# JulHoltzDevelopers/WavesAndEigenvalues.jl

Measured on AMD Instinct MI355X. Metric: eigenpairs/sec, higher is better.
Workload: dtype f64

## Files before the change

wavesandeigenvalues.jl_amd/csrc/debug.hip:

```cpp
#include <algorithm>

#include "family.h"

namespace {
struct StreamGuard {
    hipStream_t s = nullptr;
    ~StreamGuard() { if (s) (void)hipStreamDestroy(s); }
};
int64_t span(int64_t nv, int64_t stride, int64_t blk) { return nv > 0 ? (nv - 1) * stride + blk : 0; }
}

extern "C" int wae_debug_vec(int32_t device, int32_t op, const int64_t *sz, int32_t nsz, double *const *bufs, const int64_t *lens, int32_t nbuf,
                             const uint8_t *cmask, const int32_t *perm, int32_t *status_out) {
    return guarded([&]() {
        WAE_REQUIRE(sz && nsz >= 2 && nsz <= 16 && nbuf >= 0 && nbuf <= 16 && (nbuf == 0 || (bufs && lens)), "bad argument");
        int ndev = 0;
        HIP_CHECK(hipGetDeviceCount(&ndev));
        WAE_REQUIRE(device >= 0 && device < ndev, "no such device");
        for (int i = 0; i < nsz; ++i) WAE_REQUIRE(sz[i] >= 0 && sz[i] <= ((int64_t)1 << 31), "a size is negative or too large");
        for (int i = 0; i < nbuf; ++i) WAE_REQUIRE(lens[i] >= 0 && lens[i] <= ((int64_t)1 << 31), "a buffer length is negative or too large");
        auto S = [&](int i) -> int64_t { WAE_REQUIRE(i < nsz, "too few sizes for this operation"); return sz[i]; };
        WAE_REQUIRE(op != WAE_VEC_DENSE || sz[0] <= 2048, "dense coarse level too large (n > 2048)");
        HIP_CHECK(hipSetDevice(device));
        StreamGuard sg;
// ... 14 lines not shown
        const int64_t blk = n * nb;
        auto mask = [&]() -> const unsigned char * {
            if (!cmask) return nullptr;
            cm.upload(cmask, (size_t)(nb + 7) / 8, st);
            return cm.p;
        };
        auto count_of = [&](int i) -> int { const int64_t v = S(i); WAE_REQUIRE(v <= 4096, "a count is too large"); return (int)v; };
        auto want_partial = [&]() { partial.alloc((size_t)std::max(1024 * 32, 768 * 35) * (size_t)nb); return partial.p; };
        switch (op) {
        case WAE_VEC_DOTS: {
            const int nv = count_of(2);
            const int64_t stride = S(3);
            const cplx *V = need(0, span(nv, stride, blk)), *W = need(1, blk), *scale = opt(3, (int64_t)nv * nb);
            cplx *out = need(2, (int64_t)nv * nb);
            if (scale) launch_dots_scaled(V, (size_t)stride, nv, W, n, (int)nb, want_partial(), out, scale, st, mask());
            else launch_dots(V, (size_t)stride, nv, W, n, (int)nb, want_partial(), out, st, mask());
            break;
        }
        case WAE_VEC_NORMS:
            launch_norms(need(0, blk), n, (int)nb, want_partial(), need(1, nb), st, mask());
            break;
        case WAE_VEC_DOTS_MULTI: {
            const int nv = count_of(2), nw = count_of(3);
            WAE_REQUIRE(nw >= 1 && nw <= 4, "nw in 1..4");
            const cplx *V = need(0, span(nv, S(4), blk)), *W = need(1, span(nw, S(5), blk));
            launch_dots_multi(V, (size_t)S(4), nv, W, (size_t)S(5), nw, n, (int)nb, want_partial(), need(2, (int64_t)nv * nw * nb), st);
            break;
        }
        case WAE_VEC_AXPY_NEG: case WAE_VEC_LINCOMB: case WAE_VEC_LINCOMB_ADD: {
            const int nv = count_of(2);
            const cplx *V = need(0, span(nv, S(3), blk)), *c = need(1, (int64_t)nv * nb);
            cplx *W = need(2, blk);
            if (op == WAE_VEC_AXPY_NEG) launch_axpy_neg(V, (size_t)S(3), nv, c, W, n, (int)nb, st, mask());
            else if (op == WAE_VEC_LINCOMB) launch_lincomb(V, (size_t)S(3), nv, c, W, n, (int)nb, st);
            else launch_lincomb_add(V, (size_t)S(3), nv, c, W, n, (int)nb, st);
            break;
        }
        case WAE_VEC_AXPY_NEG_NORM: {
            const int nv = count_of(2);
            const cplx *V = need(0, span(nv, S(3), blk)), *h = need(1, (int64_t)nv * nb), *base = opt(4, blk);
            cplx *W = need(2, blk), *norms = need(3, nb), *inv = opt(5, nb);
            launch_axpy_neg_norm(V, (size_t)S(3), nv, h, W, n, (int)nb, want_partial(), norms, st, mask(), base, inv);
            break;
        }
        case WAE_VEC_AXPY_NEG_MULTI: {
            const int nv = count_of(2), cnt = count_of(4);
            WAE_REQUIRE(nv >= 1 && cnt >= 1 && cnt <= 4, "nv >= 1, cnt in 1..4");
            const cplx *V = need(0, span(nv, S(3), blk)), *h = need(1, (int64_t)nv * cnt * nb);
            launch_axpy_neg_multi(V, (size_t)S(3), nv, h, need(2, span(cnt, S(5), blk)), (size_t)S(5), cnt, n, (int)nb, st);
// ... 86 lines not shown
```

wavesandeigenvalues.jl_amd/csrc/family.h:

```cpp
#pragma once
#include <algorithm>
#include <chrono>
#include <future>

#include "amg.h"
#include "tiles.h"

struct RbState {
    cplx *Q = nullptr;
    int cap = 0, l = 0, S = 0;
    std::vector<int> kact;
    std::vector<zc> Hk;
    std::vector<zc> g;
    DevBuf<cplx> W, Vi, hb, alpha, alpha2, ycoef;
    std::future<void> w_job;
    void wait_w() { if (w_job.valid()) w_job.get(); }
    bool vi_valid = false;
    ~RbState() { if (w_job.valid()) w_job.wait(); }
};

struct wae_family {
    bool vc_light = false;
    int device = 0;
    hipStream_t stream = nullptr;
    int64_t d = 0;
    int T = 0;
    std::vector<int> term_plane;
    std::vector<zc> term_scale;
    std::vector<int64_t> term_nnz;
    int nplanes = 0;
    std::vector<CsrZ> planes0;
    std::vector<int> perm_h;
    DevBuf<int> perm_dev;
    std::vector<int> tile_row_ptr;
    const int *perm() const { return perm_dev.p; }
    std::vector<LevelOp> ops;
// ... 37 lines not shown
    size_t h_pin_pair_n = 0;
    size_t pc_stride_level = 0;
    ~wae_family() {
        if (stream) (void)hipStreamSynchronize(stream);
        if (h_pinned) (void)hipHostFree(h_pinned);
        if (h_pin_pair) (void)hipHostFree(h_pin_pair);
        if (stream) (void)hipStreamDestroy(stream);
    }
};

struct Batch {
    int nb;
    int cps;
    int nsys;
    int op;
};

static int env_int(const char *name, int dflt) { const char *v = getenv(name); return v ? atoi(v) : dflt; }
static bool xfer_tiles_on() { return env_int("WAE_XFER_TILES", 1) != 0; }
static double now_s() { return std::chrono::duration<double>(std::chrono::steady_clock::now().time_since_epoch()).count(); }
static void require_solver(const wae_family *h) {
    if (!h->solver_ready) throw WaeError(WAE_ERR_INVALID, "wae_solver_setup has not been called");
}
static void plane_coeffs(const wae_family *h, const double *coeffs, int op, std::vector<zc> &pc) {
    pc.assign(h->nplanes, zc(0));
    for (int k = 0; k < h->T; ++k) pc[h->term_plane[k]] += h->term_scale[k] * zc(coeffs[2 * k], coeffs[2 * k + 1]);
    if (op == WAE_OP_C)
        for (auto &c : pc) c = std::conj(c);
}

template <class F> static int guarded(F &&f) {
    try {
        return f();
    } catch (const WaeError &e) {
        wae_set_error(e.what());
        return e.code;
    } catch (const std::bad_alloc &) {
        wae_set_error("out of host memory");
        return WAE_ERR_INVALID;
    } catch (const std::exception &e) {
        wae_set_error(e.what());
        return WAE_ERR_INVALID;
    }
}
```

wavesandeigenvalues.jl_amd/csrc/lib.hip:

```cpp
#include <cmath>

#include "family.h"

static thread_local std::string g_last_error;
void wae_set_error(const std::string &m) { g_last_error = m; }

int wae_internal_device(const wae_family *h) { return h->device; }
hipStream_t wae_internal_stream(const wae_family *h) { return h->stream; }

static void upload_pc(wae_family *h, const std::vector<std::vector<zc>> &pcs) {
    const int nsys = (int)pcs.size();
    const int nl = (int)h->ops.size();
    const size_t per_level = (size_t)nsys * h->nplanes;
    std::vector<cplx> tab(per_level * (nl + 2));
    for (int l = 0; l <= nl + 1; ++l) {
        if (l >= nl && h->n_penalty == 0) break;
        const std::vector<int> &sp = l < nl ? h->slot_plane[l] : (l == nl ? h->pen_slot : h->pen_row_slot);
        for (int s = 0; s < nsys; ++s)
            for (int q = 0; q < h->nplanes; ++q) {
                const zc c = pcs[s][sp[q]];
                tab[l * per_level + (size_t)s * h->nplanes + q] = cplx{c.real(), c.imag()};
            }
    }
    h->pc_stride_level = per_level;
// ... 770 lines not shown
    for (int k = n - 1; k >= 0; --k) {
        if (dead[k]) { b[k] = 0; continue; }
        zc sres = b[k];
        for (int j = k + 1; j < n; ++j) sres -= A[(size_t)j * n + k] * b[j];
        b[k] = sres / A[(size_t)k * n + k];
    }
}

static void rb_d2h(wae_family *h, const cplx *src, cplx *dst, size_t cnt) {
    HIP_CHECK(hipMemcpyAsync(dst, src, cnt * sizeof(cplx), hipMemcpyDeviceToHost, h->stream));
    HIP_CHECK(hipStreamSynchronize(h->stream));
}

static void rb_reset(wae_family *h, cplx *Q, int cap, int l, const double *table, int npts, const cplx *Vinter) {
    RbState &R = h->rb;
    const int T = h->T;
    R.Q = Q; R.cap = cap; R.l = l; R.S = 0;
    R.kact.clear();
    for (int k = 0; k < T; ++k) {
        bool used = false;
        for (int p = 0; p < npts && !used; ++p) used = table[((size_t)p * T + k) * 2] != 0.0 || table[((size_t)p * T + k) * 2 + 1] != 0.0;
        if (used) R.kact.push_back(k);
    }
    const size_t vecl = (size_t)h->d * l;
    R.wait_w();
    if (R.W.n < R.kact.size() * (size_t)cap * vecl) {
        const size_t need = R.kact.size() * (size_t)cap * vecl;
        const int dev = h->device;
        RbState *Rp = &R;
        R.w_job = std::async(std::launch::async, [Rp, need, dev]() {
            HIP_CHECK(hipSetDevice(dev));
            Rp->W.alloc(need);
        });
    }
    R.Hk.assign(R.kact.size() * (size_t)cap * cap * l, zc(0));
    R.g.assign((size_t)cap * l, zc(0));
    if (R.Vi.n < vecl) R.Vi.alloc(vecl);
    HIP_CHECK(hipMemcpyAsync(R.Vi.p, Vinter, vecl * sizeof(cplx), hipMemcpyDeviceToDevice, h->stream));
    R.vi_valid = true;
    if (R.hb.n < (size_t)4 * (cap + 4) * l) R.hb.alloc((size_t)4 * (cap + 4) * l);
    if (R.alpha.n < (size_t)l) R.alpha.alloc(l);
    if (R.alpha2.n < (size_t)cap * l) R.alpha2.alloc((size_t)cap * l);
}

static void rb_append_block(wae_family *h, int cnt, const std::vector<std::vector<std::vector<zc>>> &pck) {
    RbState &R = h->rb;
    hipStream_t st = h->stream;
    const int64_t d = h->d;
    const int l = R.l, cap = R.cap, S = R.S;
    const size_t vecl = (size_t)d * l;
    std::vector<cplx> hh((size_t)(S + cnt) * cnt * l), n0((size_t)cnt * l), n1(l);
    const OpDev A0 = h->ops[0].dev(WAE_OP_N);
    cplx *qn = R.Q + (size_t)S * vecl;
    for (int j = 0; j < cnt; ++j) launch_norms(qn + (size_t)j * vecl, d, l, h->partial.p, R.hb.p + (size_t)j * l, st);
    rb_d2h(h, R.hb.p, n0.data(), (size_t)cnt * l);
    static const bool multi_axpy = !(getenv("WAE_RB_MULTI_AXPY") && atoi(getenv("WAE_RB_MULTI_AXPY")) == 0);
    const bool fits = (size_t)S * cnt * l * sizeof(cplx) <= 60 * 1024;
    for (int pass = 0; pass < 2 && S > 0; ++pass) {
        launch_dots_multi(R.Q, vecl, S, qn, vecl, cnt, d, l, h->partial.p, R.hb.p, st);
        if (multi_axpy && fits) {
            launch_axpy_neg_multi(R.Q, vecl, S, R.hb.p, qn, vecl, cnt, d, l, st);
            continue;
        }
        rb_d2h(h, R.hb.p, hh.data(), (size_t)S * cnt * l);
        std::vector<cplx> cj((size_t)S * l);
        for (int j = 0; j < cnt; ++j) {
            for (int i = 0; i < S; ++i)
                for (int c = 0; c < l; ++c) cj[(size_t)i * l + c] = hh[((size_t)i * cnt + j) * l + c];
            R.alpha2.upload(cj.data(), cj.size(), st);
            launch_axpy_neg(R.Q, vecl, S, R.alpha2.p, qn + (size_t)j * vecl, d, l, st);
            HIP_CHECK(hipStreamSynchronize(st));
        }
    }
    for (int j = 0; j < cnt; ++j) {
        cplx *q = qn + (size_t)j * vecl;
        for (int pass = 0; pass < 2 && j > 0; ++pass) {
            launch_dots(qn, vecl, j, q, d, l, h->partial.p, R.hb.p, st);
            launch_axpy_neg(qn, vecl, j, R.hb.p, q, d, l, st);
        }
        launch_norms(q, d, l, h->partial.p, R.hb.p, st);
        rb_d2h(h, R.hb.p, n1.data(), l);
        for (int c = 0; c < l; ++c) {
            const double nrm0 = n0[(size_t)j * l + c].x;
            n1[c] = (n1[c].x > 1e-9 * nrm0 && nrm0 > 0.0) ? cplx{n1[c].x, 0.0} : cplx{0.0, 0.0};
        }
        R.alpha.upload(n1.data(), l, st);
        launch_scale_inv(q, R.alpha.p, q, d, l, st);
        HIP_CHECK(hipStreamSynchronize(st));
    }
    launch_dots_multi(qn, vecl, cnt, R.Vi.p, vecl, 1, d, l, h->partial.p, R.hb.p, st);
    rb_d2h(h, R.hb.p, hh.data(), (size_t)cnt * l);
    for (int j = 0; j < cnt; ++j)
        for (int c = 0; c < l; ++c) R.g[(size_t)(S + j) * l + c] = zc(hh[(size_t)j * l + c].x, hh[(size_t)j * l + c].y);
    for (size_t ki = 0; ki < R.kact.size(); ++ki) {
        R.wait_w();
        cplx *Wk = R.W.p + ki * (size_t)cap * vecl;
        cplx *wn = Wk + (size_t)S * vecl;
        upload_pc(h, pck[ki]);
        for (int j = 0; j < cnt; ++j)
            launch_spmv(A0, pc_level(h, 0), l, qn + (size_t)j * vecl, wn + (size_t)j * vecl, nullptr, 0.0, l, MODE_AX, st);
        zc *H = &R.Hk[ki * (size_t)cap * cap * l];
        launch_dots_multi(R.Q, vecl, S + cnt, wn, vecl, cnt, d, l, h->partial.p, R.hb.p, st);
        rb_d2h(h, R.hb.p, hh.data(), (size_t)(S + cnt) * cnt * l);
        for (int i = 0; i < S + cnt; ++i)
            for (int j = 0; j < cnt; ++j)
                for (int c = 0; c < l; ++c) {
                    const cplx v = hh[((size_t)i * cnt + j) * l + c];
                    H[((size_t)(S + j) * cap + i) * l + c] = zc(v.x, v.y);
                }
        zc herm_factor(0);
        bool herm = false;
        {
            static const bool herm_on = !(getenv("WAE_RB_HERMITIAN") && atoi(getenv("WAE_RB_HERMITIAN")) == 0);
            const int kterm = R.kact[ki], pl = h->term_plane[kterm];
            const LevelOp &L0 = h->ops[0];
            for (size_t g = 0; g < L0.groups.size() && herm_on && !herm; ++g)
                for (int q = 0; q < L0.groups[g].nplanes; ++q)
                    if (h->slot_plane[0][(size_t)L0.groups[g].plane0 + q] == pl && L0.groups[g].symmetric && L0.groups[g].is_real) {
                        const zc sc = h->term_scale[kterm];
                        if (sc != zc(0)) { herm = true; herm_factor = sc / std::conj(sc); }
                    }
        }
        if (S > 0 && herm) {
            for (int i = 0; i < S; ++i)
                for (int j = 0; j < cnt; ++j)
                    for (int c = 0; c < l; ++c)
                        H[((size_t)i * cap + S + j) * l + c] = herm_factor * std::conj(H[((size_t)(S + j) * cap + i) * l + c]);
        } else if (S > 0) {
            launch_dots_multi(Wk, vecl, S, qn, vecl, cnt, d, l, h->partial.p, R.hb.p, st);
            rb_d2h(h, R.hb.p, hh.data(), (size_t)S * cnt * l);
            for (int i = 0; i < S; ++i)
                for (int j = 0; j < cnt; ++j)
                    for (int c = 0; c < l; ++c) {
                        const cplx v = hh[((size_t)i * cnt + j) * l + c];
                        H[((size_t)i * cap + S + j) * l + c] = zc(v.x, -v.y);
                    }
        }
    }
    R.S += cnt;
}

static void rb_append(wae_family *h, int count) {
    RbState &R = h->rb;
    WAE_REQUIRE(R.S + count <= R.cap, "snapshot store is full");
    std::vector<std::vector<std::vector<zc>>> pck(R.kact.size());
    for (size_t ki = 0; ki < R.kact.size(); ++ki) {
        std::vector<double> ek((size_t)2 * h->T, 0.0);
        ek[(size_t)2 * R.kact[ki]] = 1.0;
        pck[ki].resize(1);
        plane_coeffs(h, ek.data(), WAE_OP_N, pck[ki][0]);
    }
    for (int done = 0; done < count; done += 4) rb_append_block(h, std::min(4, count - done), pck);
}

static std::vector<cplx> rb_guess_coeffs(const wae_family *h, const double *ct_chunk, int ns) {
    const RbState &R = h->rb;
    const int S = R.S, l = R.l, cap = R.cap, T = h->T, nb = ns * l;
    std::vector<cplx> Y((size_t)S * nb);
    std::vector<zc> Hs((size_t)S * S), rhs(S);
    for (int sy = 0; sy < ns; ++sy) {
        const double *ct = ct_chunk + (size_t)sy * 2 * T;
        for (int k = 0; k < T; ++k)
            if ((ct[2 * k] != 0.0 || ct[2 * k + 1] != 0.0) && std::find(R.kact.begin(), R.kact.end(), k) == R.kact.end())
                throw WaeError(WAE_ERR_INVALID, "a term outside the projected set has a non-zero coefficient: rebuild the basis (mode 1)");
        for (int c = 0; c < l; ++c) {
            std::fill(Hs.begin(), Hs.end(), zc(0));
            for (size_t ki = 0; ki < R.kact.size(); ++ki) {
                const zc ck(ct[2 * R.kact[ki]], ct[2 * R.kact[ki] + 1]);
                if (ck == zc(0)) continue;
                const zc *H = &R.Hk[ki * (size_t)cap * cap * l];
                for (int sc = 0; sc < S; ++sc)
                    for (int i = 0; i < S; ++i) Hs[(size_t)sc * S + i] += ck * H[((size_t)sc * cap + i) * l + c];
            }
            for (int i = 0; i < S; ++i) rhs[i] = R.g[(size_t)i * l + c];
            small_solve(Hs, rhs, S);
// ... 1392 lines not shown
```

wavesandeigenvalues.jl_amd/csrc/setup.hip:

```cpp
#include <atomic>
#include <cmath>
#include <exception>
#include <map>
#include <memory>
#include <tuple>

#include "family.h"

OpDev LevelOp::dev(int op) const {
    OpDev o;
    memset(&o, 0, sizeof(o));
    o.ngroups = (int)groups.size();
    o.nplanes_total = nplanes;
    o.n = n;
    o.diag = diag.p;
    o.conj_diag = (op == WAE_OP_C) ? 1 : 0;
    o.tiles = !tiles.ready ? nullptr : (op == WAE_OP_N || tiles.all_symmetric) ? &tiles.dev : (tiles.ready_t ? &tiles.dev_t : nullptr);
    {
        const LongRows &LR = (op == WAE_OP_N) ? long_n : long_t;
        o.nlong = LR.n;
        o.long_rows = LR.rows.p; o.long_ptr = LR.ptr.p; o.long_col = LR.col.p; o.long_slot = LR.slot.p;
        o.long_val = LR.val.p; o.long_acc = LR.acc.p; o.long_part = LR.part.p;
        o.long_conj = (op == WAE_OP_C) ? 1 : 0;
    }
// ... 793 lines not shown
        h->NB = (int)opt(6, 64);
        WAE_REQUIRE(h->NB >= 1 && h->NB <= 256, "batch width must be in 1..256");
        WAE_REQUIRE(h->restart >= 2 && h->restart <= 200, "restart must be in 2..200");
        excl = (uint64_t)opt(7, 0.0);
        plane_coeffs(h, coeffs_ref, WAE_OP_N, pc);
        if (excl) {
            std::vector<double> cs(coeffs_ref, coeffs_ref + (size_t)2 * h->T);
            for (int k = 0; k < h->T && k < 52; ++k)
                if (excl >> k & 1) cs[2 * k] = cs[2 * k + 1] = 0.0;
            plane_coeffs(h, cs.data(), WAE_OP_N, pc_shape);
        }
    }

    void drop_hierarchy() {
        h->ops.resize(1);
        h->slot_plane.resize(1);
        h->xfer.clear();
    }

    void reserve_device_memory() {
        const size_t vec = (size_t)h->d * h->NB, need = vec * (size_t)(h->restart + 1);
        const size_t hint_l = (size_t)opt(8, 0.0), hint_s = (size_t)opt(9, 0.0);
        const size_t need_q = hint_l > 0 && hint_s > 0 && hint_l <= (size_t)h->NB ? (size_t)h->d * hint_l * hint_s : 0;
        const size_t need_w = need_q * (size_t)h->nplanes;
        h->rb.wait_w();
        if (h->V.n == need && h->rbQ.n >= need_q && h->rb.W.n >= need_w) return;
        basis_job.f = std::async(std::launch::async, [this, need, need_q, need_w]() {
            HIP_CHECK(hipSetDevice(h->device));
            if (h->V.n != need) h->V.alloc(need);
            const bool new_q = h->rbQ.n < need_q, new_w = h->rb.W.n < need_w;
            if (new_q) h->rbQ.alloc(need_q);
            if (new_w) h->rb.W.alloc(need_w);
            if (new_q && need_q) HIP_CHECK(hipMemset(h->rbQ.p, 0, need_q * sizeof(cplx)));
            if (new_w && need_w) HIP_CHECK(hipMemset(h->rb.W.p, 0, need_w * sizeof(cplx)));
            HIP_CHECK(hipDeviceSynchronize());
        });
    }

    void coarsen() {
        std::vector<int> visit0;
        if (!h->perm_h.empty()) { visit0.resize(h->perm_h.size()); for (size_t i = 0; i < h->perm_h.size(); ++i) visit0[h->perm_h[i]] = (int)i; }
        const bool want_plan = env.tile_level1 && !h->tile_row_ptr.empty();
        amg_setup(h->planes0, pc, ao, lv, &pen, excl ? &pc_shape : nullptr, visit0.empty() ? nullptr : &visit0, [&](const AmgLevel &L) {
            if (!want_plan || l1_job.f.valid() || &L != &lv[0]) return;
            l1_job.f = std::async(std::launch::async, [this]() { l1.run(h, lv[0], env); });
        });
        t_amg1 = now_s();
// ... 147 lines not shown
```

wavesandeigenvalues.jl_amd/csrc/vec.hip:

```cpp
#include "kernel_helpers.h"

__global__ void fill_zero_kernel(cplx *X, size_t count) {
    for (size_t e = (size_t)blockIdx.x * 256 + threadIdx.x; e < count; e += (size_t)gridDim.x * 256) X[e] = cplx{0.0, 0.0};
}
void launch_fill_zero(cplx *X, size_t count, hipStream_t st) {
    if (!count) return;
    hipLaunchKernelGGL(fill_zero_kernel, dim3(grid_for(count)), dim3(256), 0, st, X, count);
    HIP_CHECK(hipGetLastError());
}
void launch_copy(const cplx *X, cplx *Y, size_t count, hipStream_t st) {
    if (!count) return;
    HIP_CHECK(hipMemcpyAsync(Y, X, count * sizeof(cplx), hipMemcpyDeviceToDevice, st));
}
__global__ void add_kernel(const cplx *__restrict__ X, cplx *__restrict__ Y, size_t count) {
    for (size_t e = (size_t)blockIdx.x * 256 + threadIdx.x; e < count; e += (size_t)gridDim.x * 256) {
        cplx a = X[e], b = Y[e];
        Y[e] = cplx{a.x + b.x, a.y + b.y};
    }
}
void launch_add(const cplx *X, cplx *Y, size_t count, hipStream_t st) {
    if (!count) return;
    hipLaunchKernelGGL(add_kernel, dim3(grid_for(count)), dim3(256), 0, st, X, Y, count);
    HIP_CHECK(hipGetLastError());
}

__device__ __forceinline__ cplx vadd(cplx a, cplx b) { return cplx{a.x + b.x, a.y + b.y}; }
__device__ __forceinline__ double vadd(double a, double b) { return a + b; }
__device__ __forceinline__ cplx vshfl_xor(cplx a, int m) { return cplx{__shfl_xor(a.x, m), __shfl_xor(a.y, m)}; }
__device__ __forceinline__ double vshfl_xor(double a, int m) { return __shfl_xor(a, m); }
template <bool POW2, int NT, class T>
__device__ __forceinline__ T block_colsum(T v, int nb, T *sm) {
    const int tid = threadIdx.x;
    if (POW2) {
        for (int m = 32; m >= nb; m >>= 1) v = vadd(v, vshfl_xor(v, m));
        if ((tid & 63) < nb) sm[(tid >> 6) * nb + (tid & 63)] = v;
    } else {
        sm[tid] = v;
    }
    __syncthreads();
    if (tid < nb) {
        const int terms = POW2 ? NT / 64 : NT / nb;
        v = sm[tid];
        for (int k = 1; k < terms; ++k) v = vadd(v, sm[k * nb + tid]);
    }
    __syncthreads();
    return v;
}
template <int EPB>
__device__ __forceinline__ cplx sum_partials(const cplx *__restrict__ partial, int nblk, int count) {
    __shared__ cplx sm[256];
    constexpr int NS = 256 / EPB;
    const int slice = threadIdx.x / EPB;
    const int e = blockIdx.x * EPB + threadIdx.x % EPB;
    cplx acc = {0.0, 0.0};
    if (e < count)
        for (int k = slice; k < nblk; k += NS) { const cplx p = partial[(size_t)k * count + e]; acc.x += p.x; acc.y += p.y; }
    sm[threadIdx.x] = acc;
    __syncthreads();
#pragma unroll
    for (int s = NS / 2; s >= 1; s >>= 1) {
        if (slice < s) { sm[threadIdx.x].x += sm[threadIdx.x + s * EPB].x; sm[threadIdx.x].y += sm[threadIdx.x + s * EPB].y; }
        __syncthreads();
    }
    return sm[threadIdx.x];
}

constexpr int DOT_BLOCKS = 1024;
template <int MAXV, bool POW2>
__global__ __launch_bounds__(256) void dots_kernel(const cplx *__restrict__ V, size_t stride, int nv, const cplx *__restrict__ W,
                                                   int64_t n, int nb, cplx *__restrict__ partial,
// ... 92 lines not shown
            for (int i = 0; i < MAXV; ++i) {
                if (i < nv) {
                    const cplx v = V[(size_t)i * sv + e];
#pragma unroll
                    for (int j = 0; j < NW; ++j) {
                        acc[i][j].x += v.x * w[j].x + v.y * w[j].y;
                        acc[i][j].y += v.x * w[j].y - v.y * w[j].x;
                    }
                }
            }
        }
    }
#pragma unroll
    for (int i = 0; i < MAXV; ++i) {
#pragma unroll
        for (int j = 0; j < NW; ++j) {
            if (i < nv && j < nw) {
                const cplx s = block_colsum<false, 256>(acc[i][j], nb, sm);
                if (tid < nb) partial[((size_t)blockIdx.x * nv * nw + (size_t)i * nw + j) * nb + tid] = s;
            }
        }
    }
}
void launch_dots_multi(const cplx *V, size_t sv, int nv, const cplx *W, size_t sw, int nw, int64_t n, int nb, cplx *partial, cplx *out,
                       hipStream_t st) {
    if (nb < 1 || nb > 256 || nw < 1 || nw > 4) throw WaeError(WAE_ERR_INVALID, "dots_multi: nb in 1..256, nw in 1..4");
    int done = 0;
    while (done < nv) {
        const int chunk = std::min(8, nv - done);
        const int nblk = 768;
        hipLaunchKernelGGL((dots_multi_kernel<8, 4>), dim3(nblk), dim3(256), 0, st, V + (size_t)done * sv, sv, chunk, W, sw, nw, n, nb, partial);
        HIP_CHECK(hipGetLastError());
        const int count = chunk * nw * nb;
        launch_reduce_partials(partial, nblk, count, out + (size_t)done * nw * nb, 0, st);
        done += chunk;
    }
}
void launch_dots(const cplx *V, size_t stride, int nv, const cplx *W, int64_t n, int nb, cplx *partial, cplx *out, hipStream_t st,
                 const unsigned char *cmask) {
    dots_impl(V, stride, nv, W, n, nb, partial, out, 0, st, cmask);
}
void launch_dots_scaled(const cplx *V, size_t stride, int nv, const cplx *W, int64_t n, int nb, cplx *partial, cplx *out, const cplx *scale,
                        hipStream_t st, const unsigned char *cmask) {
    dots_impl(V, stride, nv, W, n, nb, partial, out, 0, st, cmask, scale);
}
void launch_norms(const cplx *X, int64_t n, int nb, cplx *partial, cplx *out, hipStream_t st, const unsigned char *cmask) {
    dots_impl(X, 0, 1, X, n, nb, partial, out, 1, st, cmask);
}

// ... 405 lines not shown
                               n, nb, l, nsys, done ? 1 : 0);
        });
        return;
    }
    const unsigned grid = row_grid(n, nb, 256, 1, 2048).grid;
    for_coef_groups(nv, nb, [&](int done, int chunk, size_t shm) {
        hipLaunchKernelGGL(lincomb_rep_kernel, dim3(grid), dim3(256), shm, st, Q + (size_t)done * stride, stride, chunk, y + (size_t)done * nb, X, n,
                           nb, l, done ? 1 : 0);
    });
}
__global__ __launch_bounds__(256) void mask_cols_kernel(cplx *__restrict__ X, const cplx *__restrict__ keep, size_t total, int nb) {
    for (size_t e = (size_t)blockIdx.x * 256 + threadIdx.x; e < total; e += (size_t)gridDim.x * 256) {
        if (keep[e % nb].x == 0.0) X[e] = cplx{0.0, 0.0};
    }
}
void launch_mask_cols(cplx *X, const cplx *keep, int64_t n, int nb, hipStream_t st) {
    const size_t total = (size_t)n * nb;
    if (!total) return;
    hipLaunchKernelGGL(mask_cols_kernel, dim3(grid_for(total)), dim3(256), 0, st, X, keep, total, nb);
    HIP_CHECK(hipGetLastError());
}

__global__ __launch_bounds__(256) void scale_inv_kernel(const cplx *__restrict__ X, const cplx *__restrict__ alpha, cplx *__restrict__ Y, size_t total, int nb,
                                                        const unsigned char *__restrict__ cmask) {
    for (size_t e = (size_t)blockIdx.x * 256 + threadIdx.x; e < total; e += (size_t)gridDim.x * 256) {
        if (cmask && !cmask[(e % nb) >> 3]) continue;
        const double a = alpha[e % nb].x;
        const double s = (a > 1e-300) ? 1.0 / a : 0.0;
        const cplx x = X[e];
        Y[e] = cplx{x.x * s, x.y * s};
    }
}
void launch_scale_inv(const cplx *X, const cplx *alpha, cplx *Y, int64_t n, int nb, hipStream_t st, const unsigned char *cmask) {
    size_t total = (size_t)n * nb;
    if (!total) return;
    hipLaunchKernelGGL(scale_inv_kernel, dim3(grid_for(total)), dim3(256), 0, st, X, alpha, Y, total, nb, cmask);
    HIP_CHECK(hipGetLastError());
}

__global__ __launch_bounds__(256) void axpby1_kernel(cplx a, const cplx *x, cplx b, const cplx *y, cplx *out, size_t n, int conj_x) {
    for (size_t e = (size_t)blockIdx.x * 256 + threadIdx.x; e < n; e += (size_t)gridDim.x * 256) {
        cplx r = cmul(a, conj_x ? cconj(x[e]) : x[e]);
        cfma(r, b, y[e]);
        out[e] = r;
    }
}
void launch_axpby1(cplx a, const cplx *x, cplx b, const cplx *y, cplx *out, size_t n, hipStream_t st, int conj_x) {
    if (!n) return;
    hipLaunchKernelGGL(axpby1_kernel, dim3(grid_for(n)), dim3(256), 0, st, a, x, b, y, out, n, conj_x);
    HIP_CHECK(hipGetLastError());
}
__global__ __launch_bounds__(256) void colmajor_to_inter_kernel(const cplx *__restrict__ Xc, int64_t d, int r, cplx *__restrict__ Xi, int nb,
                                                                const int *__restrict__ perm) {
    const size_t total = (size_t)d * nb;
    for (size_t e = (size_t)blockIdx.x * 256 + threadIdx.x; e < total; e += (size_t)gridDim.x * 256) {
        const size_t row = e / nb;
        const int b = (int)(e - row * nb);
        const size_t src = perm ? (size_t)perm[row] : row;
        Xi[e] = (b < r) ? Xc[(size_t)b * d + src] : cplx{0.0, 0.0};
// ... 427 lines not shown
```

wavesandeigenvalues.jl_amd/csrc/wae_internal.h:

```cpp
#pragma once
#include <hip/hip_runtime.h>
#include <complex>
#include <cstdint>
#include <cstdio>
#include <cstring>
#include <stdexcept>
#include <string>
#include <vector>

#include "../../include/waehip.h"

typedef std::complex<double> zc;
typedef double2 cplx;

struct WaeError : std::runtime_error {
    int code;
    WaeError(int c, const std::string &m) : std::runtime_error(m), code(c) {}
};
void wae_set_error(const std::string &m);
int wae_internal_device(const wae_family *h);
hipStream_t wae_internal_stream(const wae_family *h);

#define HIP_CHECK(expr)                                                                                  \
    do {                                                                                                 \
// ... 192 lines not shown
void launch_jacobi0(const OpDev &op, const cplx *pc, int cps, const cplx *B, cplx *X, double jac_w, int nb, hipStream_t s,
                    const unsigned char *cmask = nullptr);
void launch_spmv_multi(const OpDev &op, const cplx *pc, const int *plane_col, const cplx *X, cplx *Y, int nb, hipStream_t s);

void launch_dense_assemble(const cplx *planes, int nplanes, int n, const cplx *pc, int nsys, int op,
                           cplx *Ainv, hipStream_t s);
void launch_dense_invert(cplx *Ainv, int n, int nsys, int *status, hipStream_t s);
void launch_dense_apply(const cplx *Ainv, int n, int cps, const cplx *X, cplx *Y, int nb, hipStream_t s, const unsigned char *cmask = nullptr);

void launch_fill_zero(cplx *X, size_t count, hipStream_t s);
void launch_copy(const cplx *X, cplx *Y, size_t count, hipStream_t s);
void launch_dots(const cplx *V, size_t stride, int nv, const cplx *W, int64_t n, int nb, cplx *partial, cplx *out, hipStream_t s,
                 const unsigned char *cmask = nullptr);
void launch_axpy_neg_multi(const cplx *V, size_t stride, int nv, const cplx *h, cplx *W, size_t wstride, int cnt, int64_t n, int nb, hipStream_t s);
void launch_axpy_neg(const cplx *V, size_t stride, int nv, const cplx *h, cplx *W, int64_t n, int nb, hipStream_t s,
                     const unsigned char *cmask = nullptr);
void launch_axpy_neg_norm(const cplx *V, size_t stride, int nv, const cplx *h, cplx *W, int64_t n, int nb, cplx *partial, cplx *norms,
                          hipStream_t s, const unsigned char *cmask = nullptr, const cplx *base = nullptr, cplx *inv_out = nullptr);
void launch_dots_scaled(const cplx *V, size_t stride, int nv, const cplx *W, int64_t n, int nb, cplx *partial, cplx *out, const cplx *scale,
                        hipStream_t s, const unsigned char *cmask = nullptr);
void launch_lincomb(const cplx *V, size_t stride, int nv, const cplx *y, cplx *Y, int64_t n, int nb, hipStream_t s);
void launch_lincomb_add(const cplx *V, size_t stride, int nv, const cplx *y, cplx *X, int64_t n, int nb, hipStream_t s);
void launch_norms(const cplx *X, int64_t n, int nb, cplx *partial, cplx *out, hipStream_t s, const unsigned char *cmask = nullptr);
void launch_scale_inv(const cplx *X, const cplx *alpha, cplx *Y, int64_t n, int nb, hipStream_t s, const unsigned char *cmask = nullptr);
void launch_axpby1(cplx a, const cplx *x, cplx b, const cplx *y, cplx *out, size_t n, hipStream_t s, int conj_x = 0);
void launch_add(const cplx *X, cplx *Y, size_t count, hipStream_t s);
void launch_colmajor_to_inter(const cplx *Xc, int64_t d, int r, cplx *Xi, int nb, hipStream_t s, const int *perm = nullptr);
void launch_inter_to_colmajor(const cplx *Xi, int nb, int64_t d, int r, cplx *Xc, hipStream_t s, const int *perm = nullptr);
void launch_replicate(const cplx *Vc, int64_t d, int l, cplx *Xi, int nb, hipStream_t s, const int *perm = nullptr);
void launch_prolong_add(const int *ptr, const int *col, const double *val, int64_t n, const cplx *Xc, cplx *X, int nb, hipStream_t s,
                        const unsigned char *cmask = nullptr);
void launch_dots_multi(const cplx *V, size_t sv, int nv, const cplx *W, size_t sw, int nw, int64_t n, int nb, cplx *partial, cplx *out,
                       hipStream_t s);
void launch_gather_rows(const cplx *X, const int *rows, int64_t nrows, int nb, cplx *out, hipStream_t s);
void launch_scatter_add_rows(const cplx *D, const int *rows, int64_t nrows, int nb, cplx *X, hipStream_t s);
void launch_extract_cols(const cplx *X, int nb, int off, int l, cplx *out, int64_t n, hipStream_t s);
void launch_lincomb_rep(const cplx *Q, size_t stride, int nv, const cplx *y, cplx *X, int64_t n, int nb, int l, hipStream_t s);
void launch_mask_cols(cplx *X, const cplx *keep, int64_t n, int nb, hipStream_t s);
void launch_beyn_accum(const cplx *Xi, int nb, int64_t d, int l, int nsys, const cplx *w, const cplx *z, int npow, cplx *A, hipStream_t s,
                       int lA = 0, int c0 = 0, const int *perm = nullptr);
void launch_pt_gemm_batch(const cplx *V, size_t stride, int k, const cplx *G, cplx *U, int64_t d, int T, int nb, hipStream_t s);
void launch_pt_spmv_batch(const OpDev &op, const cplx *pc, const int *plane_col, const cplx *U, int nin, cplx *Y, int nb, int accumulate,
                          hipStream_t s);
void launch_pt_axpby_cols(const cplx *coef, const cplx *x, const cplx *y, cplx *out, int64_t d, int nb, hipStream_t s);
void launch_pt_project(cplx *vk, const cplx *v0, const cplx *dots, int nd, int64_t d, int nb, hipStream_t s);
struct GmresDev {
    int nb, m, histcap;
    cplx *R;
    double *cs;
    cplx *sn;
    cplx *g;
    double *sv;
    cplx *vsq;
    int *conv, *steps, *iters, *histlen, *stalled;
    double *relres, *bnorm;
    double *hist;
// ... 17 lines not shown
```

Before: 4.364.

## Batch reduced-basis append projections and remove host round-trips

Restructures the reduced-basis snapshot append so the spmv results for up to four terms, together with the initial-vector projection, are projected against Q by a single new wide multi-RHS dots kernel. All results come back in one device-to-host copy instead of one per term. The norm thresholding moves into scale_inv on the device, which removes per-column syncs and uploads. For Hermitian terms, W storage keeps only the current block rather than the whole basis, which cuts memory. This adds a new kernel with larger partial buffers and more complex bookkeeping, and the non-fitting axpy path now allocates a temporary device buffer on every pass.

```diff
diff --git a/wavesandeigenvalues.jl_amd/csrc/debug.hip b/wavesandeigenvalues.jl_amd/csrc/debug.hip
--- a/wavesandeigenvalues.jl_amd/csrc/debug.hip
+++ b/wavesandeigenvalues.jl_amd/csrc/debug.hip
@@ -60,9 +60,10 @@
             break;
         case WAE_VEC_DOTS_MULTI: {
             const int nv = count_of(2), nw = count_of(3);
-            WAE_REQUIRE(nw >= 1 && nw <= 4, "nw in 1..4");
+            WAE_REQUIRE(nw >= 1 && nw <= DOTS_MAXW, "nw in 1..20");
             const cplx *V = need(0, span(nv, S(4), blk)), *W = need(1, span(nw, S(5), blk));
-            launch_dots_multi(V, (size_t)S(4), nv, W, (size_t)S(5), nw, n, (int)nb, want_partial(), need(2, (int64_t)nv * nw * nb), st);
+            partial.alloc(dots_multi_partial_count(nw, (int)nb));
+            launch_dots_multi(V, (size_t)S(4), nv, W, (size_t)S(5), nw, n, (int)nb, partial.p, need(2, (int64_t)nv * nw * nb), st);
             break;
         }
         case WAE_VEC_AXPY_NEG: case WAE_VEC_LINCOMB: case WAE_VEC_LINCOMB_ADD: {
diff --git a/wavesandeigenvalues.jl_amd/csrc/family.h b/wavesandeigenvalues.jl_amd/csrc/family.h
--- a/wavesandeigenvalues.jl_amd/csrc/family.h
+++ b/wavesandeigenvalues.jl_amd/csrc/family.h
@@ -12,6 +12,8 @@
     std::vector<int> kact;
     std::vector<zc> Hk;
     std::vector<zc> g;
+    std::vector<zc> herm;
+    std::vector<size_t> woff;
     DevBuf<cplx> W, Vi, hb, alpha, alpha2, ycoef;
     std::future<void> w_job;
     void wait_w() { if (w_job.valid()) w_job.get(); }
@@ -95,6 +97,22 @@
 static void require_solver(const wae_family *h) {
     if (!h->solver_ready) throw WaeError(WAE_ERR_INVALID, "wae_solver_setup has not been called");
 }
+constexpr int RB_BLOCK = 4;
+constexpr int RB_TERMS = 4;
+static bool plane_real_symmetric(const wae_family *h, int pl) {
+    const LevelOp &L0 = h->ops[0];
+    for (size_t g = 0; g < L0.groups.size(); ++g)
+        for (int q = 0; q < L0.groups[g].nplanes; ++q)
+            if (h->slot_plane[0][(size_t)L0.groups[g].plane0 + q] == pl && L0.groups[g].symmetric && L0.groups[g].is_real) return true;
+    return false;
+}
+static bool rb_term_hermitian(const wae_family *h, int kterm, zc *factor) {
+    static const bool herm_on = env_int("WAE_RB_HERMITIAN", 1) != 0;
+    const zc sc = h->term_scale[kterm];
+    if (!herm_on || sc == zc(0) || !plane_real_symmetric(h, h->term_plane[kterm])) return false;
+    *factor = sc / std::conj(sc);
+    return true;
+}
 static void plane_coeffs(const wae_family *h, const double *coeffs, int op, std::vector<zc> &pc) {
     pc.assign(h->nplanes, zc(0));
     for (int k = 0; k < h->T; ++k) pc[h->term_plane[k]] += h->term_scale[k] * zc(coeffs[2 * k], coeffs[2 * k + 1]);
diff --git a/wavesandeigenvalues.jl_amd/csrc/lib.hip b/wavesandeigenvalues.jl_amd/csrc/lib.hip
--- a/wavesandeigenvalues.jl_amd/csrc/lib.hip
+++ b/wavesandeigenvalues.jl_amd/csrc/lib.hip
@@ -816,10 +816,16 @@
         for (int p = 0; p < npts && !used; ++p) used = table[((size_t)p * T + k) * 2] != 0.0 || table[((size_t)p * T + k) * 2 + 1] != 0.0;
         if (used) R.kact.push_back(k);
     }
-    const size_t vecl = (size_t)h->d * l;
+    const size_t vecl = (size_t)h->d * l, nk = R.kact.size();
+    R.herm.assign(nk, zc(0));
+    R.woff.assign(nk, 0);
+    size_t need = 0;
+    for (size_t ki = 0; ki < nk; ++ki) {
+        R.woff[ki] = need;
+        need += (size_t)(rb_term_hermitian(h, R.kact[ki], &R.herm[ki]) ? RB_BLOCK : cap) * vecl;
+    }
     R.wait_w();
-    if (R.W.n < R.kact.size() * (size_t)cap * vecl) {
-        const size_t need = R.kact.size() * (size_t)cap * vecl;
+    if (R.W.n < need) {
         const int dev = h->device;
         RbState *Rp = &R;
         R.w_job = std::async(std::launch::async, [Rp, need, dev]() {
@@ -827,27 +833,29 @@
             Rp->W.alloc(need);
         });
     }
-    R.Hk.assign(R.kact.size() * (size_t)cap * cap * l, zc(0));
+    R.Hk.assign(nk * (size_t)cap * cap * l, zc(0));
     R.g.assign((size_t)cap * l, zc(0));
     if (R.Vi.n < vecl) R.Vi.alloc(vecl);
     HIP_CHECK(hipMemcpyAsync(R.Vi.p, Vinter, vecl * sizeof(cplx), hipMemcpyDeviceToDevice, h->stream));
     R.vi_valid = true;
-    if (R.hb.n < (size_t)4 * (cap + 4) * l) R.hb.alloc((size_t)4 * (cap + 4) * l);
+    const size_t hbn = (2 * nk * RB_BLOCK + 1) * (size_t)(cap + RB_BLOCK) * l;
+    if (R.hb.n < hbn) R.hb.alloc(hbn);
     if (R.alpha.n < (size_t)l) R.alpha.alloc(l);
     if (R.alpha2.n < (size_t)cap * l) R.alpha2.alloc((size_t)cap * l);
-}
-
-static void rb_append_block(wae_family *h, int cnt, const std::vector<std::vector<std::vector<zc>>> &pck) {
+    const size_t np = dots_multi_partial_count(RB_TERMS * RB_BLOCK + 1, l);
+    if (h->partial.n < np) h->partial.alloc(np);
+}
+
+static void rb_append_block(wae_family *h, int cnt) {
     RbState &R = h->rb;
     hipStream_t st = h->stream;
     const int64_t d = h->d;
     const int l = R.l, cap = R.cap, S = R.S;
-    const size_t vecl = (size_t)d * l;
-    std::vector<cplx> hh((size_t)(S + cnt) * cnt * l), n0((size_t)cnt * l), n1(l);
+    const size_t vecl = (size_t)d * l, nk = R.kact.size();
     const OpDev A0 = h->ops[0].dev(WAE_OP_N);
     cplx *qn = R.Q + (size_t)S * vecl;
-    for (int j = 0; j < cnt; ++j) launch_norms(qn + (size_t)j * vecl, d, l, h->partial.p, R.hb.p + (size_t)j * l, st);
-    rb_d2h(h, R.hb.p, n0.data(), (size_t)cnt * l);
+    cplx *n0 = R.alpha2.p;
+    for (int j = 0; j < cnt; ++j) launch_norms(qn + (size_t)j * vecl, d, l, h->partial.p, n0 + (size_t)j * l, st);
     static const bool multi_axpy = !(getenv("WAE_RB_MULTI_AXPY") && atoi(getenv("WAE_RB_MULTI_AXPY")) == 0);
     const bool fits = (size_t)S * cnt * l * sizeof(cplx) <= 60 * 1024;
     for (int pass = 0; pass < 2 && S > 0; ++pass) {
@@ -856,13 +864,14 @@
             launch_axpy_neg_multi(R.Q, vecl, S, R.hb.p, qn, vecl, cnt, d, l, st);
             continue;
         }
-        rb_d2h(h, R.hb.p, hh.data(), (size_t)S * cnt * l);
-        std::vector<cplx> cj((size_t)S * l);
+        std::vector<cplx> hh((size_t)S * cnt * l), cj((size_t)S * l);
+        rb_d2h(h, R.hb.p, hh.data(), hh.size());
+        DevBuf<cplx> cdev;
         for (int j = 0; j < cnt; ++j) {
             for (int i = 0; i < S; ++i)
                 for (int c = 0; c < l; ++c) cj[(size_t)i * l + c] = hh[((size_t)i * cnt + j) * l + c];
-            R.alpha2.upload(cj.data(), cj.size(), st);
-            launch_axpy_neg(R.Q, vecl, S, R.alpha2.p, qn + (size_t)j * vecl, d, l, st);
+            cdev.upload(cj.data(), cj.size(), st);
+            launch_axpy_neg(R.Q, vecl, S, cdev.p, qn + (size_t)j * vecl, d, l, st);
             HIP_CHECK(hipStreamSynchronize(st));
         }
     }
@@ -872,79 +881,76 @@
             launch_dots(qn, vecl, j, q, d, l, h->partial.p, R.hb.p, st);
             launch_axpy_neg(qn, vecl, j, R.hb.p, q, d, l, st);
         }
-        launch_norms(q, d, l, h->partial.p, R.hb.p, st);
-        rb_d2h(h, R.hb.p, n1.data(), l);
+        launch_norms(q, d, l, h->partial.p, R.alpha.p, st);
+        launch_scale_inv(q, R.alpha.p, q, d, l, st, nullptr, n0 + (size_t)j * l);
+    }
+    R.wait_w();
+    const int nq = S + cnt;
+    struct Round { size_t ki0, nkr, off; int nw; };
+    std::vector<Round> rounds;
+    size_t nget = 0;
+    for (size_t ki0 = 0; ki0 < nk || ki0 == 0; ki0 += RB_TERMS) {
+        const size_t nkr = std::min<size_t>(RB_TERMS, nk - ki0);
+        const cplx *rhs[DOTS_MAXW];
+        int nw = 0;
+        for (size_t ki = ki0; ki < ki0 + nkr; ++ki) {
+            cplx *wn = R.W.p + R.woff[ki] + (R.herm[ki] != zc(0) ? 0 : (size_t)S * vecl);
+            for (int j = 0; j < cnt; ++j) {
+                launch_spmv(A0, pc_level(h, 0) + ki * (size_t)h->nplanes, l, qn + (size_t)j * vecl, wn + (size_t)j * vecl, nullptr, 0.0, l, MODE_AX, st);
+                rhs[nw++] = wn + (size_t)j * vecl;
+            }
+        }
+        if (ki0 == 0) rhs[nw++] = R.Vi.p;
+        launch_dots_multi_list(R.Q, vecl, nq, rhs, nw, d, l, h->partial.p, R.hb.p + nget, st);
+        rounds.push_back({ki0, nkr, nget, nw});
+        nget += (size_t)nq * nw * l;
+    }
+    const size_t nrow = (size_t)S * cnt * l, rows0 = nget;
+    for (size_t ki = 0; ki < nk && S > 0; ++ki)
+        if (R.herm[ki] == zc(0)) {
+            launch_dots_multi(R.W.p + R.woff[ki], vecl, S, qn, vecl, cnt, d, l, h->partial.p, R.hb.p + nget, st);
+            nget += nrow;
+        }
+    std::vector<cplx> hh(nget);
+    rb_d2h(h, R.hb.p, hh.data(), nget);
+    for (int j = 0; j < cnt; ++j)
         for (int c = 0; c < l; ++c) {
-            const double nrm0 = n0[(size_t)j * l + c].x;
-            n1[c] = (n1[c].x > 1e-9 * nrm0 && nrm0 > 0.0) ? cplx{n1[c].x, 0.0} : cplx{0.0, 0.0};
-        }
-        R.alpha.upload(n1.data(), l, st);
-        launch_scale_inv(q, R.alpha.p, q, d, l, st);
-        HIP_CHECK(hipStreamSynchronize(st));
-    }
-    launch_dots_multi(qn, vecl, cnt, R.Vi.p, vecl, 1, d, l, h->partial.p, R.hb.p, st);
-    rb_d2h(h, R.hb.p, hh.data(), (size_t)cnt * l);
-    for (int j = 0; j < cnt; ++j)
-        for (int c = 0; c < l; ++c) R.g[(size_t)(S + j) * l + c] = zc(hh[(size_t)j * l + c].x, hh[(size_t)j * l + c].y);
-    for (size_t ki = 0; ki < R.kact.size(); ++ki) {
-        R.wait_w();
-        cplx *Wk = R.W.p + ki * (size_t)cap * vecl;
-        cplx *wn = Wk + (size_t)S * vecl;
-        upload_pc(h, pck[ki]);
-        for (int j = 0; j < cnt; ++j)
-            launch_spmv(A0, pc_level(h, 0), l, qn + (size_t)j * vecl, wn + (size_t)j * vecl, nullptr, 0.0, l, MODE_AX, st);
-        zc *H = &R.Hk[ki * (size_t)cap * cap * l];
-        launch_dots_multi(R.Q, vecl, S + cnt, wn, vecl, cnt, d, l, h->partial.p, R.hb.p, st);
-        rb_d2h(h, R.hb.p, hh.data(), (size_t)(S + cnt) * cnt * l);
-        for (int i = 0; i < S + cnt; ++i)
-            for (int j = 0; j < cnt; ++j)
-                for (int c = 0; c < l; ++c) {
-                    const cplx v = hh[((size_t)i * cnt + j) * l + c];
-                    H[((size_t)(S + j) * cap + i) * l + c] = zc(v.x, v.y);
-                }
-        zc herm_factor(0);
-        bool herm = false;
-        {
-            static const bool herm_on = !(getenv("WAE_RB_HERMITIAN") && atoi(getenv("WAE_RB_HERMITIAN")) == 0);
-            const int kterm = R.kact[ki], pl = h->term_plane[kterm];
-            const LevelOp &L0 = h->ops[0];
-            for (size_t g = 0; g < L0.groups.size() && herm_on && !herm; ++g)
-                for (int q = 0; q < L0.groups[g].nplanes; ++q)
-                    if (h->slot_plane[0][(size_t)L0.groups[g].plane0 + q] == pl && L0.groups[g].symmetric && L0.groups[g].is_real) {
-                        const zc sc = h->term_scale[kterm];
-                        if (sc != zc(0)) { herm = true; herm_factor = sc / std::conj(sc); }
+            const cplx v = hh[((size_t)(S + j) * rounds[0].nw + rounds[0].nw - 1) * l + c];
+            R.g[(size_t)(S + j) * l + c] = zc(v.x, v.y);
+        }
+    const cplx *rows = hh.data() + rows0;
+    for (const Round &rd : rounds)
+        for (size_t ki = rd.ki0; ki < rd.ki0 + rd.nkr; ++ki) {
+            zc *H = &R.Hk[ki * (size_t)cap * cap * l];
+            for (int i = 0; i < nq; ++i)
+                for (int j = 0; j < cnt; ++j)
+                    for (int c = 0; c < l; ++c) {
+                        const cplx v = hh[rd.off + ((size_t)i * rd.nw + (ki - rd.ki0) * cnt + j) * l + c];
+                        H[((size_t)(S + j) * cap + i) * l + c] = zc(v.x, v.y);
                     }
-        }
-        if (S > 0 && herm) {
+            if (S == 0) continue;
+            const bool herm = R.herm[ki] != zc(0);
             for (int i = 0; i < S; ++i)
                 for (int j = 0; j < cnt; ++j)
                     for (int c = 0; c < l; ++c)
-                        H[((size_t)i * cap + S + j) * l + c] = herm_factor * std::conj(H[((size_t)(S + j) * cap + i) * l + c]);
-        } else if (S > 0) {
-            launch_dots_multi(Wk, vecl, S, qn, vecl, cnt, d, l, h->partial.p, R.hb.p, st);
-            rb_d2h(h, R.hb.p, hh.data(), (size_t)S * cnt * l);
-            for (int i = 0; i < S; ++i)
-                for (int j = 0; j < cnt; ++j)
-                    for (int c = 0; c < l; ++c) {
-                        const cplx v = hh[((size_t)i * cnt + j) * l + c];
-                        H[((size_t)i * cap + S + j) * l + c] = zc(v.x, -v.y);
-                    }
-        }
-    }
+                        H[((size_t)i * cap + S + j) * l + c] = herm ? R.herm[ki] * std::conj(H[((size_t)(S + j) * cap + i) * l + c])
+                                                                    : std::conj(zc(rows[((size_t)i * cnt + j) * l + c].x, rows[((size_t)i * cnt + j) * l + c].y));
+            if (!herm) rows += nrow;
+        }
     R.S += cnt;
 }
 
 static void rb_append(wae_family *h, int count) {
     RbState &R = h->rb;
     WAE_REQUIRE(R.S + count <= R.cap, "snapshot store is full");
-    std::vector<std::vector<std::vector<zc>>> pck(R.kact.size());
+    std::vector<std::vector<zc>> pck(R.kact.size());
     for (size_t ki = 0; ki < R.kact.size(); ++ki) {
         std::vector<double> ek((size_t)2 * h->T, 0.0);
         ek[(size_t)2 * R.kact[ki]] = 1.0;
-        pck[ki].resize(1);
-        plane_coeffs(h, ek.data(), WAE_OP_N, pck[ki][0]);
-    }
-    for (int done = 0; done < count; done += 4) rb_append_block(h, std::min(4, count - done), pck);
+        plane_coeffs(h, ek.data(), WAE_OP_N, pck[ki]);
+    }
+    if (!pck.empty()) upload_pc(h, pck);
+    for (int done = 0; done < count; done += RB_BLOCK) rb_append_block(h, std::min(RB_BLOCK, count - done));
 }
 
 static std::vector<cplx> rb_guess_coeffs(const wae_family *h, const double *ct_chunk, int ns) {
diff --git a/wavesandeigenvalues.jl_amd/csrc/setup.hip b/wavesandeigenvalues.jl_amd/csrc/setup.hip
--- a/wavesandeigenvalues.jl_amd/csrc/setup.hip
+++ b/wavesandeigenvalues.jl_amd/csrc/setup.hip
@@ -839,7 +839,8 @@
         const size_t vec = (size_t)h->d * h->NB, need = vec * (size_t)(h->restart + 1);
         const size_t hint_l = (size_t)opt(8, 0.0), hint_s = (size_t)opt(9, 0.0);
         const size_t need_q = hint_l > 0 && hint_s > 0 && hint_l <= (size_t)h->NB ? (size_t)h->d * hint_l * hint_s : 0;
-        const size_t need_w = need_q * (size_t)h->nplanes;
+        size_t need_w = 0;
+        for (int pl = 0; pl < h->nplanes && need_q; ++pl) need_w += (size_t)h->d * hint_l * (plane_real_symmetric(h, pl) ? (size_t)RB_BLOCK : hint_s);
         h->rb.wait_w();
         if (h->V.n == need && h->rbQ.n >= need_q && h->rb.W.n >= need_w) return;
         basis_job.f = std::async(std::launch::async, [this, need, need_q, need_w]() {
diff --git a/wavesandeigenvalues.jl_amd/csrc/vec.hip b/wavesandeigenvalues.jl_amd/csrc/vec.hip
--- a/wavesandeigenvalues.jl_amd/csrc/vec.hip
+++ b/wavesandeigenvalues.jl_amd/csrc/vec.hip
@@ -29,8 +29,7 @@
 __device__ __forceinline__ cplx vshfl_xor(cplx a, int m) { return cplx{__shfl_xor(a.x, m), __shfl_xor(a.y, m)}; }
 __device__ __forceinline__ double vshfl_xor(double a, int m) { return __shfl_xor(a, m); }
 template <bool POW2, int NT, class T>
-__device__ __forceinline__ T block_colsum(T v, int nb, T *sm) {
-    const int tid = threadIdx.x;
+__device__ __forceinline__ T block_colsum(T v, int nb, T *sm, const int tid) {
     if (POW2) {
         for (int m = 32; m >= nb; m >>= 1) v = vadd(v, vshfl_xor(v, m));
         if ((tid & 63) < nb) sm[(tid >> 6) * nb + (tid & 63)] = v;
@@ -46,6 +45,8 @@
     __syncthreads();
     return v;
 }
+template <bool POW2, int NT, class T>
+__device__ __forceinline__ T block_colsum(T v, int nb, T *sm) { return block_colsum<POW2, NT>(v, nb, sm, (int)threadIdx.x); }
 template <int EPB>
 __device__ __forceinline__ cplx sum_partials(const cplx *__restrict__ partial, int nblk, int count) {
     __shared__ cplx sm[256];
@@ -184,9 +185,101 @@
         }
     }
 }
+constexpr int DW_MAXV = 8, DW_NWT = 5;
+constexpr int DW_BLOCKS = 512;
+struct DotsRhs { const cplx *p[DOTS_MAXW]; };
+template <int G, int NV>
+__device__ __forceinline__ void dots_wide_rows(const cplx *__restrict__ V, size_t sv, const cplx *(&Wp)[DW_NWT], int nwg, int64_t n, int nb,
+                                               int b, int rl, cplx (&acc)[DW_MAXV][DW_NWT]) {
+    const int R = (256 / G) / nb;
+    for (int64_t row = (int64_t)blockIdx.x * R + rl; row < n; row += (int64_t)gridDim.x * R) {
+        const size_t e = (size_t)row * nb + b;
+        cplx w[DW_NWT], v[NV];
+#pragma unroll
+        for (int j = 0; j < DW_NWT; ++j) w[j] = j < nwg ? Wp[j][e] : cplx{0.0, 0.0};
+#pragma unroll
+        for (int i = 0; i < NV; ++i) v[i] = stream_load(V + (size_t)i * sv + e);
+#pragma unroll
+        for (int i = 0; i < NV; ++i)
+#pragma unroll
+            for (int j = 0; j < DW_NWT; ++j) {
+                acc[i][j].x += v[i].x * w[j].x + v[i].y * w[j].y;
+                acc[i][j].y += v[i].x * w[j].y - v[i].y * w[j].x;
+            }
+    }
+}
+template <int G>
+__global__ __launch_bounds__(256) void dots_wide_kernel(const cplx *__restrict__ V, size_t sv, int nv, DotsRhs W, int nw, int jd, int nwt,
+                                                        int64_t n, int nb, cplx *__restrict__ partial) {
+    constexpr int TPG = 256 / G;
+    __shared__ cplx sm[256];
+    const int g = threadIdx.x / TPG, t = threadIdx.x % TPG;
+    const int b = t % nb, rl = t / nb;
+    const int j0 = g * DW_NWT;
+    const int nwg = nw - j0 < DW_NWT ? nw - j0 : DW_NWT;
+    const cplx *Wp[DW_NWT];
+#pragma unroll
+    for (int j = 0; j < DW_NWT; ++j) Wp[j] = W.p[j < nwg ? j0 + j : 0];
+    cplx acc[DW_MAXV][DW_NWT];
+#pragma unroll
+    for (int i = 0; i < DW_MAXV; ++i)
+#pragma unroll
+        for (int j = 0; j < DW_NWT; ++j) acc[i][j] = cplx{0.0, 0.0};
+    if (rl < TPG / nb && nwg > 0) {
+        switch (nv) {
+        case 1: dots_wide_rows<G, 1>(V, sv, Wp, nwg, n, nb, b, rl, acc); break;
+        case 2: dots_wide_rows<G, 2>(V, sv, Wp, nwg, n, nb, b, rl, acc); break;
+        case 3: dots_wide_rows<G, 3>(V, sv, Wp, nwg, n, nb, b, rl, acc); break;
+        case 4: dots_wide_rows<G, 4>(V, sv, Wp, nwg, n, nb, b, rl, acc); break;
+        case 5: dots_wide_rows<G, 5>(V, sv, Wp, nwg, n, nb, b, rl, acc); break;
+        case 6: dots_wide_rows<G, 6>(V, sv, Wp, nwg, n, nb, b, rl, acc); break;
+        case 7: dots_wide_rows<G, 7>(V, sv, Wp, nwg, n, nb, b, rl, acc); break;
+        default: dots_wide_rows<G, 8>(V, sv, Wp, nwg, n, nb, b, rl, acc); break;
+        }
+    }
+    const bool pow2 = nb <= 64 && (nb & (nb - 1)) == 0;
+#pragma unroll
+    for (int i = 0; i < DW_MAXV; ++i) {
+        if (i < nv) {
+#pragma unroll
+            for (int j = 0; j < DW_NWT; ++j) {
+                const cplx s = pow2 ? block_colsum<true, TPG>(acc[i][j], nb, sm + g * TPG, t) : block_colsum<false, TPG>(acc[i][j], nb, sm + g * TPG, t);
+                if (t < nb && j < nwg) partial[((size_t)blockIdx.x * nv * nwt + (size_t)i * nwt + jd + j0 + j) * nb + t] = s;
+            }
+        }
+    }
+}
+size_t dots_multi_partial_count(int nw, int nb) { return (size_t)(nw <= 4 ? 768 * DW_MAXV * 4 : DW_BLOCKS * DW_MAXV * nw) * (size_t)nb; }
+void launch_dots_multi_list(const cplx *V, size_t sv, int nv, const cplx *const *W, int nw, int64_t n, int nb, cplx *partial, cplx *out,
+                            hipStream_t st) {
+    if (nb < 1 || nb > 256 || nw < 1 || nw > DOTS_MAXW) throw WaeError(WAE_ERR_INVALID, "dots_multi: nb in 1..256, nw in 1..20");
+    const int G = nw <= DW_NWT || nb > 128 ? 1 : (nw <= 2 * DW_NWT || nb > 64 ? 2 : 4);
+    const int R = 256 / G / nb;
+    const int nblk = (int)std::min<int64_t>(DW_BLOCKS, (n + R - 1) / R);
+    for (int done = 0; done < nv; done += DW_MAXV) {
+        const int chunk = std::min(DW_MAXV, nv - done);
+        const cplx *Vc = V + (size_t)done * sv;
+        for (int jd = 0; jd < nw; jd += G * DW_NWT) {
+            DotsRhs rhs{};
+            const int nwc = std::min(G * DW_NWT, nw - jd);
+            for (int j = 0; j < nwc; ++j) rhs.p[j] = W[jd + j];
+            if (G == 1) hipLaunchKernelGGL(dots_wide_kernel<1>, dim3(nblk), dim3(256), 0, st, Vc, sv, chunk, rhs, nwc, jd, nw, n, nb, partial);
+            else if (G == 2) hipLaunchKernelGGL(dots_wide_kernel<2>, dim3(nblk), dim3(256), 0, st, Vc, sv, chunk, rhs, nwc, jd, nw, n, nb, partial);
+            else hipLaunchKernelGGL(dots_wide_kernel<4>, dim3(nblk), dim3(256), 0, st, Vc, sv, chunk, rhs, nwc, jd, nw, n, nb, partial);
+            HIP_CHECK(hipGetLastError());
+        }
+        launch_reduce_partials(partial, nblk, chunk * nw * nb, out + (size_t)done * nw * nb, 0, st);
+    }
+}
 void launch_dots_multi(const cplx *V, size_t sv, int nv, const cplx *W, size_t sw, int nw, int64_t n, int nb, cplx *partial, cplx *out,
                        hipStream_t st) {
-    if (nb < 1 || nb > 256 || nw < 1 || nw > 4) throw WaeError(WAE_ERR_INVALID, "dots_multi: nb in 1..256, nw in 1..4");
+    if (nb < 1 || nb > 256 || nw < 1 || nw > DOTS_MAXW) throw WaeError(WAE_ERR_INVALID, "dots_multi: nb in 1..256, nw in 1..20");
+    if (nw > 4) {
+        const cplx *Wp[DOTS_MAXW];
+        for (int j = 0; j < nw; ++j) Wp[j] = W + (size_t)j * sw;
+        launch_dots_multi_list(V, sv, nv, Wp, nw, n, nb, partial, out, st);
+        return;
+    }
     int done = 0;
     while (done < nv) {
         const int chunk = std::min(8, nv - done);
@@ -638,19 +731,20 @@
 }
 
 __global__ __launch_bounds__(256) void scale_inv_kernel(const cplx *__restrict__ X, const cplx *__restrict__ alpha, cplx *__restrict__ Y, size_t total, int nb,
-                                                        const unsigned char *__restrict__ cmask) {
+                                                        const unsigned char *__restrict__ cmask, const cplx *__restrict__ ref) {
     for (size_t e = (size_t)blockIdx.x * 256 + threadIdx.x; e < total; e += (size_t)gridDim.x * 256) {
         if (cmask && !cmask[(e % nb) >> 3]) continue;
         const double a = alpha[e % nb].x;
-        const double s = (a > 1e-300) ? 1.0 / a : 0.0;
+        double s = (a > 1e-300) ? 1.0 / a : 0.0;
+        if (ref) { const double r = ref[e % nb].x; if (!(a > 1e-9 * r && r > 0.0)) s = 0.0; }
         const cplx x = X[e];
         Y[e] = cplx{x.x * s, x.y * s};
     }
 }
-void launch_scale_inv(const cplx *X, const cplx *alpha, cplx *Y, int64_t n, int nb, hipStream_t st, const unsigned char *cmask) {
+void launch_scale_inv(const cplx *X, const cplx *alpha, cplx *Y, int64_t n, int nb, hipStream_t st, const unsigned char *cmask, const cplx *ref) {
     size_t total = (size_t)n * nb;
     if (!total) return;
-    hipLaunchKernelGGL(scale_inv_kernel, dim3(grid_for(total)), dim3(256), 0, st, X, alpha, Y, total, nb, cmask);
+    hipLaunchKernelGGL(scale_inv_kernel, dim3(grid_for(total)), dim3(256), 0, st, X, alpha, Y, total, nb, cmask, ref);
     HIP_CHECK(hipGetLastError());
 }
 
diff --git a/wavesandeigenvalues.jl_amd/csrc/wae_internal.h b/wavesandeigenvalues.jl_amd/csrc/wae_internal.h
--- a/wavesandeigenvalues.jl_amd/csrc/wae_internal.h
+++ b/wavesandeigenvalues.jl_amd/csrc/wae_internal.h
@@ -238,7 +238,8 @@
 void launch_lincomb(const cplx *V, size_t stride, int nv, const cplx *y, cplx *Y, int64_t n, int nb, hipStream_t s);
 void launch_lincomb_add(const cplx *V, size_t stride, int nv, const cplx *y, cplx *X, int64_t n, int nb, hipStream_t s);
 void launch_norms(const cplx *X, int64_t n, int nb, cplx *partial, cplx *out, hipStream_t s, const unsigned char *cmask = nullptr);
-void launch_scale_inv(const cplx *X, const cplx *alpha, cplx *Y, int64_t n, int nb, hipStream_t s, const unsigned char *cmask = nullptr);
+void launch_scale_inv(const cplx *X, const cplx *alpha, cplx *Y, int64_t n, int nb, hipStream_t s, const unsigned char *cmask = nullptr,
+                      const cplx *ref = nullptr);
 void launch_axpby1(cplx a, const cplx *x, cplx b, const cplx *y, cplx *out, size_t n, hipStream_t s, int conj_x = 0);
 void launch_add(const cplx *X, cplx *Y, size_t count, hipStream_t s);
 void launch_colmajor_to_inter(const cplx *Xc, int64_t d, int r, cplx *Xi, int nb, hipStream_t s, const int *perm = nullptr);
@@ -246,8 +247,12 @@
 void launch_replicate(const cplx *Vc, int64_t d, int l, cplx *Xi, int nb, hipStream_t s, const int *perm = nullptr);
 void launch_prolong_add(const int *ptr, const int *col, const double *val, int64_t n, const cplx *Xc, cplx *X, int nb, hipStream_t s,
                         const unsigned char *cmask = nullptr);
+constexpr int DOTS_MAXW = 20;
+size_t dots_multi_partial_count(int nw, int nb);
 void launch_dots_multi(const cplx *V, size_t sv, int nv, const cplx *W, size_t sw, int nw, int64_t n, int nb, cplx *partial, cplx *out,
                        hipStream_t s);
+void launch_dots_multi_list(const cplx *V, size_t sv, int nv, const cplx *const *W, int nw, int64_t n, int nb, cplx *partial, cplx *out,
+                            hipStream_t s);
 void launch_gather_rows(const cplx *X, const int *rows, int64_t nrows, int nb, cplx *out, hipStream_t s);
 void launch_scatter_add_rows(const cplx *D, const int *rows, int64_t nrows, int nb, cplx *X, hipStream_t s);
 void launch_extract_cols(const cplx *X, int nb, int off, int l, cplx *out, int64_t n, hipStream_t s);
```

New measurement: 4.391 (median of 6 runs). About the same (+0.6%).
